# frgfm/Holocron

Measured on NVIDIA H100. Metric: images/sec RepVGG-A0 224^2 bf16 train, higher is better.
Workload: dtype bf16

## Files before the change

holocron_b200/csrc/conv_wgrad.cu:

```cuda
#include <cstdlib>
#include "conv_common.cuh"

namespace {

using namespace tc;
using namespace conv;

constexpr int kBKpix = 64;
constexpr int kChunkBytes = kBKpix * 128;
constexpr int kABytes = 2 * kChunkBytes;

struct WgradParams {
  int m_total, Ho, Wo, stride, pad, dil, R, S, Cin, Cout;
  int ci_tile;
  int ci_chunks;
  int taps_per_group;
  int num_tap_groups, num_co_tiles, num_ci_tiles, k_splits;
  int kblocks_total;
  int stages, stage_bytes;
  int use_atomics;
  float* dw;
  float* ws;
  long long dw_elems;
};

template <int CIW>
__global__ void __launch_bounds__(kThreads, 1)
conv_wgrad_kernel(const __grid_constant__ CUtensorMap tmDY, const __grid_constant__ CUtensorMap tmX, const WgradParams p) {
  constexpr int kChunks = (CIW + 63) / 64, kNLast = CIW - 64 * (kChunks - 1);
  extern __shared__ __align__(1024) uint8_t smem_raw[];
  uint8_t* smem = reinterpret_cast<uint8_t*>((reinterpret_cast<uintptr_t>(smem_raw) + 1023) & ~uintptr_t(1023));
  uint64_t* full_bar = reinterpret_cast<uint64_t*>(smem + (size_t)p.stages * p.stage_bytes);
  uint64_t* empty_bar = full_bar + p.stages;

  const int warp = threadIdx.x >> 5, lane = threadIdx.x & 31;
  if (warp == 0 && lane == 0) {
    prefetch_tmap(&tmDY);
    prefetch_tmap(&tmX);
    for (int i = 0; i < p.stages; ++i) { mbar_init(&full_bar[i], 1); mbar_init(&empty_bar[i], kConsumers / 32); }
    fence_barrier_init();
  }
  __syncthreads();

  const int RS = p.R * p.S;
  const int num_units = p.num_co_tiles * p.num_ci_tiles * p.num_tap_groups * p.k_splits;
  const int b_tap_bytes = p.ci_chunks * kChunkBytes;

  auto decode = [&](int unit, int& co_t, int& ci_t, int& tg, int& ks) {
    ks = unit % p.k_splits; unit /= p.k_splits;
    tg = unit % p.num_tap_groups; unit /= p.num_tap_groups;
    ci_t = unit % p.num_ci_tiles; co_t = unit / p.num_ci_tiles;
  };
  auto kb_range = [&](int ks, int& kb0, int& kb1) {
    const int per = (p.kblocks_total + p.k_splits - 1) / p.k_splits;
    kb0 = ks * per;
    kb1 = min(kb0 + per, p.kblocks_total);
  };

  if (warp < 4) {
    if (warp == 0 && lane == 0) {
      Ring ring;
      for (int unit = blockIdx.x; unit < num_units; unit += gridDim.x) {
        int co_t, ci_t, tg, ks, kb0, kb1;
        decode(unit, co_t, ci_t, tg, ks);
        kb_range(ks, kb0, kb1);
        const int tap0 = tg * p.taps_per_group;
        const int ntaps = min(p.taps_per_group, RS - tap0);
        const uint32_t tx = kABytes + ntaps * b_tap_bytes;
        for (int kb = kb0; kb < kb1; ++kb) {
          const int m0 = kb * kBKpix;
          const int q0 = m0 % p.Wo, p0 = (m0 / p.Wo) % p.Ho, n0 = m0 / (p.Wo * p.Ho);
          const int base_w = q0 * p.stride - p.pad, base_h = p0 * p.stride - p.pad;
          uint64_t* bar = &full_bar[ring.stage];
          mbar_wait(&empty_bar[ring.stage], ring.phase ^ 1);
          uint8_t* sa = smem + (size_t)ring.stage * p.stage_bytes;
          mbar_arrive_expect_tx(bar, tx);
          tma_load_2d(&tmDY, bar, sa, co_t * 128, m0);
          tma_load_2d(&tmDY, bar, sa + kChunkBytes, co_t * 128 + 64, m0);
          for (int t = 0; t < ntaps; ++t) {
            const int tap = tap0 + t, r = tap / p.S, s = tap % p.S;
            uint8_t* sb = sa + kABytes + t * b_tap_bytes;
            for (int c = 0; c < p.ci_chunks; ++c)
              tma_load_im2col_4d(&tmX, bar, sb + c * kChunkBytes, ci_t * p.ci_tile + c * 64, base_w, base_h, n0,
                                 (uint16_t)(s * p.dil), (uint16_t)(r * p.dil));
          }
          ring.next(p.stages);
        }
      }
    }
    return;
  }

  const int et = threadIdx.x - 128;
  const int wg = et >> 7;
  const int frow = frag_row(et & 127), fcol = frag_col(et & 127);
  const uint32_t dhi = desc_hi(1024);
  float acc[CIW / 2];
  Ring ring;
  for (int unit = blockIdx.x; unit < num_units; unit += gridDim.x) {
    int co_t, ci_t, tg, ks, kb0, kb1;
    decode(unit, co_t, ci_t, tg, ks);
    kb_range(ks, kb0, kb1);
    const int tap = tg * p.taps_per_group;
    int prev = -1;
    for (int kb = kb0; kb < kb1; ++kb) {
      mbar_wait(&full_bar[ring.stage], ring.phase);
      const uint32_t s_lo = desc_lo(smem_u32(smem + (size_t)ring.stage * p.stage_bytes), 16);
      const uint32_t a_lo = s_lo + (uint32_t)wg * (kChunkBytes >> 4);
      const uint32_t b_lo = s_lo + (kABytes >> 4);
      const uint32_t acc0 = kb > kb0 ? 1u : 0u;
      wgmma_fence();
#pragma unroll
      for (int k = 0; k < kBKpix / 16; ++k) {
        const uint64_t ad = make_desc(a_lo + k * (2048 >> 4), dhi);
        const uint32_t sc = acc0 | (uint32_t)k;
        if constexpr (kChunks == 1) {
          wgmma<kNLast, 1, 1>(acc, ad, make_desc(b_lo + k * (2048 >> 4), dhi), sc);
        } else {
          wgmma<64, 1, 1>(acc, ad, make_desc(b_lo + k * (2048 >> 4), dhi), sc);
          wgmma<kNLast, 1, 1>(acc + 32, ad, make_desc(b_lo + (kChunkBytes >> 4) + k * (2048 >> 4), dhi), sc);
        }
      }
      wgmma_commit();
      wgmma_wait<1>();
      if (prev >= 0 && lane == 0) mbar_arrive(&empty_bar[prev]);
      prev = ring.stage;
      ring.next(p.stages);
    }
    wgmma_wait<0>();
    fence_regs(acc);
    if (prev >= 0 && lane == 0) mbar_arrive(&empty_bar[prev]);

    const bool have = kb1 > kb0;
    if (!have && p.use_atomics != 2) continue;
    float* base = p.use_atomics == 2 ? p.ws + (size_t)ks * p.dw_elems : p.dw;
#pragma unroll
    for (int h = 0; h < 2; ++h) {
      const int co = co_t * 128 + 64 * wg + frow + 8 * h;
      if (co >= p.Cout) continue;
      float* drow = base + ((size_t)co * RS + tap) * p.Cin;
#pragma unroll
      for (int j = 0; j < CIW / 8; ++j) {
        const int c = (j >> 3) * 64 + 8 * (j & 7) + fcol;
        const int ci = ci_t * p.ci_tile + c;
        if (c >= p.ci_tile || ci >= p.Cin) continue;
        const float v0 = have ? acc[4 * j + 2 * h] : 0.f, v1 = have ? acc[4 * j + 2 * h + 1] : 0.f;
        if (p.use_atomics == 1) {
          atomicAdd(drow + ci, v0);
          atomicAdd(drow + ci + 1, v1);
        } else {
          *reinterpret_cast<float2*>(drow + ci) = make_float2(v0, v1);
        }
      }
    }
  }
}

__global__ void __launch_bounds__(256) wgrad_reduce_kernel(const float* __restrict__ ws, float* __restrict__ dw, long long n,
                                                           int k_splits, float* __restrict__ dw2, long long n_first,
                                                           int accumulate) {
  __shared__ float4 part[8][32];
  const long long i4 = ((long long)blockIdx.x * 32 + threadIdx.x) * 4;
  const int y = threadIdx.y;
  float4 acc = make_float4(0.f, 0.f, 0.f, 0.f);
  if (i4 + 3 < n) {
#pragma unroll 4
    for (int k = y; k < k_splits; k += 8) {
      const float4 v = *reinterpret_cast<const float4*>(ws + (size_t)k * n + i4);
      acc.x += v.x; acc.y += v.y; acc.z += v.z; acc.w += v.w;
    }
  } else if (i4 < n) {
    float t[4] = {0.f, 0.f, 0.f, 0.f};
    for (int k = y; k < k_splits; k += 8)
      for (int j = 0; j < 4 && i4 + j < n; ++j) t[j] += ws[(size_t)k * n + i4 + j];
    acc = make_float4(t[0], t[1], t[2], t[3]);
  }
  part[y][threadIdx.x] = acc;
  __syncthreads();
  if (y == 0 && i4 < n) {
    float4 r = part[0][threadIdx.x];
#pragma unroll
    for (int j = 1; j < 8; ++j) {
      const float4 v = part[j][threadIdx.x];
      r.x += v.x; r.y += v.y; r.z += v.z; r.w += v.w;
    }
    float* dst = i4 < n_first ? dw + i4 : dw2 + (i4 - n_first);
    if (i4 + 3 < n) {
      if (accumulate) {
        const float4 o = *reinterpret_cast<const float4*>(dst);
        r.x += o.x; r.y += o.y; r.z += o.z; r.w += o.w;
      }
      *reinterpret_cast<float4*>(dst) = r;
    } else {
      const float t[4] = {r.x, r.y, r.z, r.w};
      for (int j = 0; j < 4 && i4 + j < n; ++j) dst[j] = accumulate ? dst[j] + t[j] : t[j];
    }
  }
}

inline void launch_wgrad_reduce(const float* ws, float* dw, long long n, int slices, cudaStream_t st, float* dw2 = nullptr,
                                long long n_first = -1, int accumulate = 0) {
  const unsigned blocks = (unsigned)((n / 4 + 32) / 32);
  if (n_first < 0 || !dw2) { n_first = n; dw2 = dw; }
  wgrad_reduce_kernel<<<blocks, dim3(32, 8), 0, st>>>(ws, dw, n, slices, dw2, n_first, accumulate);
}

struct WgradPlan {
  WgradParams p;
  size_t ws_bytes;
};

int plan_wgrad(WgradPlan& plan, int N, int H, int W, int Cin, int Cout, int R, int S, int stride, int pad, int dil,
               int num_ctas) {
  WgradParams& p = plan.p;
  const int Ho = (H + 2 * pad - dil * (R - 1) - 1) / stride + 1;
  const int Wo = (W + 2 * pad - dil * (S - 1) - 1) / stride + 1;
  const long long m_ll = (long long)N * Ho * Wo;
  if (Ho <= 0 || Wo <= 0 || m_ll > 0x7fffffffLL) return (int)cudaErrorInvalidValue;
  p.m_total = (int)m_ll; p.Ho = Ho; p.Wo = Wo; p.stride = stride; p.pad = pad; p.dil = dil;
  p.R = R; p.S = S; p.Cin = Cin; p.Cout = Cout;
  const int RS = R * S;
  int ci_tile = Cin;
  if (Cin > 128) {
    ci_tile = 128;
    if (Cin % 128 != 0 && Cin % 64 == 0) ci_tile = 64;
  }
  p.ci_tile = ci_tile;
  p.ci_chunks = (ci_tile + 63) / 64;
  p.taps_per_group = 1;
  p.stage_bytes = kABytes + p.ci_chunks * kChunkBytes;
  p.stages = (200 * 1024) / p.stage_bytes;
  if (p.stages > 6) p.stages = 6;
  p.num_tap_groups = (RS + p.taps_per_group - 1) / p.taps_per_group;
  p.num_co_tiles = (Cout + 127) / 128;
  p.num_ci_tiles = (Cin + ci_tile - 1) / ci_tile;
  p.kblocks_total = (p.m_total + kBKpix - 1) / kBKpix;
  const int base_units = p.num_co_tiles * p.num_ci_tiles * p.num_tap_groups;
  const int ctas = num_ctas > 0 ? num_ctas : HB_NUM_SMS;
  int k_splits = (2 * ctas + base_units - 1) / base_units;
  if (base_units >= ctas) k_splits = 1;
  const int max_splits = (p.kblocks_total + 7) / 8;
  if (k_splits > max_splits) k_splits = max_splits;
  if (k_splits < 1) k_splits = 1;
  p.k_splits = k_splits;
  p.dw_elems = (long long)Cout * RS * Cin;
  plan.ws_bytes = k_splits > 1 ? (size_t)k_splits * p.dw_elems * sizeof(float) : 0;
  return 0;
}

}

extern "C" {

size_t hb_conv2d_wgrad_workspace_bytes(int N, int H, int W, int Cin, int Cout, int R, int S, int stride, int pad, int dil,
                                       int num_ctas) {
  WgradPlan plan{};
  if (plan_wgrad(plan, N, H, W, Cin, Cout, R, S, stride, pad, dil, num_ctas)) return 0;
  const size_t rows = hb_wgrad_rows_workspace_bytes(N, H, W, Cin, Cout, R, S, stride, pad, dil, num_ctas, 0);
  return rows > plan.ws_bytes ? rows : plan.ws_bytes;
}

static int wgrad_impl(const void* x, const void* dy, float* dw, float* workspace, size_t workspace_bytes, int N, int H,
                      int W, int Cin, int Cout, int R, int S, int stride, int pad, int dil, int num_ctas, void* stream,
                      int accumulate) {
  if (Cin % 8 != 0 || Cout % 8 != 0) return (int)cudaErrorInvalidValue;
  if (!hb::aligned16(x) || !hb::aligned16(dy) || !hb::aligned16(dw)) return (int)cudaErrorMisalignedAddress;
  cudaStream_t st = (cudaStream_t)stream;
  static const bool rows_enabled = getenv("HB_DISABLE_WGRAD_ROWS") == nullptr;
  if (rows_enabled && R == 3 && S == 3 && stride == 1 && pad == 1 && dil == 1 && workspace && hb::aligned16(workspace)) {
    int slices = 0;
    const int rc = hb_wgrad_rows_try(x, dy, nullptr, workspace, workspace_bytes, N, H, W, Cin, Cout, num_ctas, st, &slices);
    if (rc == 0) {
      const long long n = (long long)Cout * 9 * Cin;
      launch_wgrad_reduce(workspace, dw, n, slices, st, nullptr, -1, accumulate);
      HB_LAUNCH_CHECK();
      return 0;
    }
    if (rc != (int)cudaErrorNotSupported) return rc;
  }
  WgradPlan plan{};
  if (int rc = plan_wgrad(plan, N, H, W, Cin, Cout, R, S, stride, pad, dil, num_ctas)) return rc;
  WgradParams& p = plan.p;
  if (accumulate && !(p.k_splits > 1 && workspace && workspace_bytes >= plan.ws_bytes && hb::aligned16(workspace)))
    return (int)cudaErrorNotSupported;
  const int RS = R * S;
  const int k_splits = p.k_splits;
  const int base_units = p.num_co_tiles * p.num_ci_tiles * p.num_tap_groups;
  const int ctas = num_ctas > 0 ? num_ctas : HB_NUM_SMS;
  p.dw = dw;
  p.ws = workspace;
  if (k_splits == 1) {
    p.use_atomics = 0;
  } else if (workspace && workspace_bytes >= plan.ws_bytes && hb::aligned16(workspace)) {
    p.use_atomics = 2;
  } else {
    p.use_atomics = 1;
    cudaError_t e = cudaMemsetAsync(dw, 0, (size_t)Cout * RS * Cin * sizeof(float), st);
    if (e != cudaSuccess) return (int)e;
  }

  CUtensorMap tmDY, tmX;
  if (int rc = tmap::encode_matrix(&tmDY, dy, p.m_total, Cout, kBKpix)) return rc;
  if (int rc = tmap::encode_im2col_bf16(&tmX, x, N, H, W, Cin, pad, pad, R, S, dil, stride, 64, kBKpix,
                                        CU_TENSOR_MAP_SWIZZLE_128B))
    return rc;
  const size_t smem_bytes = (size_t)p.stages * p.stage_bytes + 2 * p.stages * sizeof(uint64_t) + 1024;
  const int num_units = base_units * k_splits;
  int grid = ctas < num_units ? ctas : num_units;
  const cudaError_t e = dispatch_width<16, 128>((p.ci_tile + 15) & ~15, [&](auto ciw) {
    return launch<conv_wgrad_kernel<decltype(ciw)::value>>(grid, smem_bytes, st, tmDY, tmX, p);
  });
  if (e != cudaSuccess) return (int)e;
  if (p.use_atomics == 2) {
    const long long n = p.dw_elems;
    launch_wgrad_reduce(workspace, dw, n, k_splits, st, nullptr, -1, accumulate);
    HB_LAUNCH_CHECK();
  }
  return 0;
}

int hb_conv2d_wgrad_bf16(const void* x, const void* dy, float* dw, float* workspace, size_t workspace_bytes, int N, int H,
                         int W, int Cin, int Cout, int R, int S, int stride, int pad, int dil, int num_ctas, void* stream) {
  return wgrad_impl(x, dy, dw, workspace, workspace_bytes, N, H, W, Cin, Cout, R, S, stride, pad, dil, num_ctas, stream, 0);
}

int hb_conv2d_wgrad_acc_bf16(const void* x, const void* dy, float* dw, float* workspace, size_t workspace_bytes, int N, int H,
                             int W, int Cin, int Cout, int R, int S, int stride, int pad, int dil, int num_ctas,
                             void* stream) {
  return wgrad_impl(x, dy, dw, workspace, workspace_bytes, N, H, W, Cin, Cout, R, S, stride, pad, dil, num_ctas, stream, 1);
}

size_t hb_repvgg_wgrad_workspace_bytes(int N, int H, int W, int Cin, int Cout, int num_ctas) {
  return hb_wgrad_rows_workspace_bytes(N, H, W, Cin, Cout, 3, 3, 1, 1, 1, num_ctas, 1);
}

static int repvgg_wgrad_impl(const void* x, const void* dy3, const void* dy1, float* dw, float* dw1, float* workspace,
                             size_t workspace_bytes, int N, int H, int W, int Cin, int Cout, int num_ctas, void* stream,
                             int accumulate) {
  if (Cin % 8 != 0 || Cout % 8 != 0) return (int)cudaErrorInvalidValue;
  if (!hb::aligned16(x) || !hb::aligned16(dy3) || !hb::aligned16(dy1) || !hb::aligned16(dw) || !hb::aligned16(workspace) ||
      !hb::aligned16(dw1))
    return (int)cudaErrorMisalignedAddress;
  cudaStream_t st = (cudaStream_t)stream;
  int slices = 0;
  if (int rc = hb_wgrad_rows_try(x, dy3, dy1, workspace, workspace_bytes, N, H, W, Cin, Cout, num_ctas, st, &slices))
    return rc;
  const long long n = (long long)Cout * 10 * Cin;
  launch_wgrad_reduce(workspace, dw, n, slices, st, dw1, dw1 ? (long long)Cout * 9 * Cin : -1, accumulate);
  HB_LAUNCH_CHECK();
  return 0;
}

int hb_repvgg_wgrad_bf16(const void* x, const void* dy3, const void* dy1, float* dw, float* workspace, size_t workspace_bytes,
                         int N, int H, int W, int Cin, int Cout, int num_ctas, void* stream) {
  return repvgg_wgrad_impl(x, dy3, dy1, dw, nullptr, workspace, workspace_bytes, N, H, W, Cin, Cout, num_ctas, stream, 0);
}

int hb_repvgg_wgrad_acc_bf16(const void* x, const void* dy3, const void* dy1, float* dw3, float* dw1, float* workspace,
                             size_t workspace_bytes, int N, int H, int W, int Cin, int Cout, int num_ctas, void* stream) {
  if (!dw1) return (int)cudaErrorInvalidValue;
  return repvgg_wgrad_impl(x, dy3, dy1, dw3, dw1, workspace, workspace_bytes, N, H, W, Cin, Cout, num_ctas, stream, 1);
}

}
```

Measured before the change: 9332.

## Use wide 192/256 input-channel tiles in wgrad with register rebalancing

Adds a wide-tile path to the weight-gradient kernel. When Cin is a multiple of 256 or 192, one CTA now covers 192 or 256 input channels with a single wide wgmma instruction, reusing each loaded dY tile across more channels and reducing redundant dY loads. The producer warps give up registers and the consumer warps take more to hold the larger accumulator, and the stage count is recomputed against the full shared-memory budget. The k-split count is still computed from the narrow unit count, and an in-kernel accumulate path lets the unsplit case add into dw directly instead of being rejected. Risks are register pressure at 232 regs per thread with a 128-float accumulator, and less parallelism from fewer ci tiles.

```diff
diff --git a/holocron_b200/csrc/conv_wgrad.cu b/holocron_b200/csrc/conv_wgrad.cu
--- a/holocron_b200/csrc/conv_wgrad.cu
+++ b/holocron_b200/csrc/conv_wgrad.cu
@@ -9,6 +9,9 @@
 constexpr int kBKpix = 64;
 constexpr int kChunkBytes = kBKpix * 128;
 constexpr int kABytes = 2 * kChunkBytes;
+constexpr int kProducerRegs = 40;
+constexpr int kConsumerRegs = 232;
+constexpr int kSmemMax = 227 * 1024;
 
 struct WgradParams {
   int m_total, Ho, Wo, stride, pad, dil, R, S, Cin, Cout;
@@ -19,6 +22,7 @@
   int kblocks_total;
   int stages, stage_bytes;
   int use_atomics;
+  int accumulate;
   float* dw;
   float* ws;
   long long dw_elems;
@@ -27,6 +31,7 @@
 template <int CIW>
 __global__ void __launch_bounds__(kThreads, 1)
 conv_wgrad_kernel(const __grid_constant__ CUtensorMap tmDY, const __grid_constant__ CUtensorMap tmX, const WgradParams p) {
+  constexpr bool kWide = CIW > 128;
   constexpr int kChunks = (CIW + 63) / 64, kNLast = CIW - 64 * (kChunks - 1);
   extern __shared__ __align__(1024) uint8_t smem_raw[];
   uint8_t* smem = reinterpret_cast<uint8_t*>((reinterpret_cast<uintptr_t>(smem_raw) + 1023) & ~uintptr_t(1023));
@@ -58,6 +63,7 @@
   };
 
   if (warp < 4) {
+    if constexpr (kWide) regs_release<kProducerRegs>();
     if (warp == 0 && lane == 0) {
       Ring ring;
       for (int unit = blockIdx.x; unit < num_units; unit += gridDim.x) {
@@ -91,6 +97,7 @@
     return;
   }
 
+  if constexpr (kWide) regs_acquire<kConsumerRegs>();
   const int et = threadIdx.x - 128;
   const int wg = et >> 7;
   const int frow = frag_row(et & 127), fcol = frag_col(et & 127);
@@ -114,7 +121,10 @@
       for (int k = 0; k < kBKpix / 16; ++k) {
         const uint64_t ad = make_desc(a_lo + k * (2048 >> 4), dhi);
         const uint32_t sc = acc0 | (uint32_t)k;
-        if constexpr (kChunks == 1) {
+        if constexpr (kWide) {
+          const uint32_t bw_lo = desc_lo(smem_u32(smem + (size_t)ring.stage * p.stage_bytes + kABytes), kChunkBytes);
+          wgmma<CIW, 1, 1>(acc, ad, make_desc(bw_lo + k * (2048 >> 4), dhi), sc);
+        } else if constexpr (kChunks == 1) {
           wgmma<kNLast, 1, 1>(acc, ad, make_desc(b_lo + k * (2048 >> 4), dhi), sc);
         } else {
           wgmma<64, 1, 1>(acc, ad, make_desc(b_lo + k * (2048 >> 4), dhi), sc);
@@ -144,12 +154,17 @@
         const int c = (j >> 3) * 64 + 8 * (j & 7) + fcol;
         const int ci = ci_t * p.ci_tile + c;
         if (c >= p.ci_tile || ci >= p.Cin) continue;
-        const float v0 = have ? acc[4 * j + 2 * h] : 0.f, v1 = have ? acc[4 * j + 2 * h + 1] : 0.f;
+        float v0 = have ? acc[4 * j + 2 * h] : 0.f, v1 = have ? acc[4 * j + 2 * h + 1] : 0.f;
         if (p.use_atomics == 1) {
           atomicAdd(drow + ci, v0);
           atomicAdd(drow + ci + 1, v1);
         } else {
-          *reinterpret_cast<float2*>(drow + ci) = make_float2(v0, v1);
+          float2* dst = reinterpret_cast<float2*>(drow + ci);
+          if (p.accumulate) {
+            const float2 o = *dst;
+            v0 = o.x + v0; v1 = o.y + v1;
+          }
+          *dst = make_float2(v0, v1);
         }
       }
     }
@@ -220,25 +235,32 @@
   p.m_total = (int)m_ll; p.Ho = Ho; p.Wo = Wo; p.stride = stride; p.pad = pad; p.dil = dil;
   p.R = R; p.S = S; p.Cin = Cin; p.Cout = Cout;
   const int RS = R * S;
-  int ci_tile = Cin;
+  int narrow = Cin;
   if (Cin > 128) {
-    ci_tile = 128;
-    if (Cin % 128 != 0 && Cin % 64 == 0) ci_tile = 64;
-  }
+    narrow = 128;
+    if (Cin % 128 != 0 && Cin % 64 == 0) narrow = 64;
+  }
+  const int wide = Cin % 256 == 0 ? 256 : Cin % 192 == 0 ? 192 : 0;
+  const int ci_tile = wide ? wide : narrow;
   p.ci_tile = ci_tile;
   p.ci_chunks = (ci_tile + 63) / 64;
   p.taps_per_group = 1;
   p.stage_bytes = kABytes + p.ci_chunks * kChunkBytes;
-  p.stages = (200 * 1024) / p.stage_bytes;
-  if (p.stages > 6) p.stages = 6;
+  if (wide) {
+    p.stages = (kSmemMax - 1024 - 2 * 8 * (int)sizeof(uint64_t)) / p.stage_bytes;
+    if (p.stages > 8) p.stages = 8;
+  } else {
+    p.stages = (200 * 1024) / p.stage_bytes;
+    if (p.stages > 6) p.stages = 6;
+  }
   p.num_tap_groups = (RS + p.taps_per_group - 1) / p.taps_per_group;
   p.num_co_tiles = (Cout + 127) / 128;
   p.num_ci_tiles = (Cin + ci_tile - 1) / ci_tile;
   p.kblocks_total = (p.m_total + kBKpix - 1) / kBKpix;
-  const int base_units = p.num_co_tiles * p.num_ci_tiles * p.num_tap_groups;
+  const int narrow_units = p.num_co_tiles * ((Cin + narrow - 1) / narrow) * p.num_tap_groups;
   const int ctas = num_ctas > 0 ? num_ctas : HB_NUM_SMS;
-  int k_splits = (2 * ctas + base_units - 1) / base_units;
-  if (base_units >= ctas) k_splits = 1;
+  int k_splits = (2 * ctas + narrow_units - 1) / narrow_units;
+  if (narrow_units >= ctas) k_splits = 1;
   const int max_splits = (p.kblocks_total + 7) / 8;
   if (k_splits > max_splits) k_splits = max_splits;
   if (k_splits < 1) k_splits = 1;
@@ -281,7 +303,7 @@
   WgradPlan plan{};
   if (int rc = plan_wgrad(plan, N, H, W, Cin, Cout, R, S, stride, pad, dil, num_ctas)) return rc;
   WgradParams& p = plan.p;
-  if (accumulate && !(p.k_splits > 1 && workspace && workspace_bytes >= plan.ws_bytes && hb::aligned16(workspace)))
+  if (accumulate && p.k_splits > 1 && !(workspace && workspace_bytes >= plan.ws_bytes && hb::aligned16(workspace)))
     return (int)cudaErrorNotSupported;
   const int RS = R * S;
   const int k_splits = p.k_splits;
@@ -289,6 +311,7 @@
   const int ctas = num_ctas > 0 ? num_ctas : HB_NUM_SMS;
   p.dw = dw;
   p.ws = workspace;
+  p.accumulate = k_splits == 1 ? accumulate : 0;
   if (k_splits == 1) {
     p.use_atomics = 0;
   } else if (workspace && workspace_bytes >= plan.ws_bytes && hb::aligned16(workspace)) {
@@ -307,9 +330,12 @@
   const size_t smem_bytes = (size_t)p.stages * p.stage_bytes + 2 * p.stages * sizeof(uint64_t) + 1024;
   const int num_units = base_units * k_splits;
   int grid = ctas < num_units ? ctas : num_units;
-  const cudaError_t e = dispatch_width<16, 128>((p.ci_tile + 15) & ~15, [&](auto ciw) {
-    return launch<conv_wgrad_kernel<decltype(ciw)::value>>(grid, smem_bytes, st, tmDY, tmX, p);
-  });
+  const cudaError_t e =
+      p.ci_tile == 256 ? launch<conv_wgrad_kernel<256>>(grid, smem_bytes, st, tmDY, tmX, p)
+      : p.ci_tile == 192 ? launch<conv_wgrad_kernel<192>>(grid, smem_bytes, st, tmDY, tmX, p)
+      : dispatch_width<16, 128>((p.ci_tile + 15) & ~15, [&](auto ciw) {
+          return launch<conv_wgrad_kernel<decltype(ciw)::value>>(grid, smem_bytes, st, tmDY, tmX, p);
+        });
   if (e != cudaSuccess) return (int)e;
   if (p.use_atomics == 2) {
     const long long n = p.dw_elems;
```

New measurement: 9499, median of 6. +1.8%, better.
